# QuentinFuxa/WhisperLiveKit

Measured on AMD Instinct MI355X. Metric: audio seconds transcribed per second (1/RTF), Whisper-base EN simul_whisper AlignAtt, 0.5 s chunks, higher is better.
Workload: dtype f32; 1 GPU; base.en simul_whisper, 1 stream(s) over 1 GPU(s) (1 per GPU), 30 s 16 kHz speech-like stream, 0.5 s chunks, beam 1, frame_threshold 25, seeded random weights, synthetic vocabulary; model=base.en, streams_total=1

## Files before the change

### include/wlk_hip.h

```cpp
#ifndef WLK_HIP_H
#define WLK_HIP_H

#include <stdint.h>

#ifdef __cplusplus
extern "C" {
#endif

#define WLK_OK 0
#define WLK_ERR_ARG (-1)
#define WLK_ERR_HIP (-2)
#define WLK_ERR_STATE (-3)
#define WLK_ERR_CAPACITY (-4)

typedef struct wlk_model wlk_model;
typedef struct wlk_session wlk_session;

typedef struct wlk_dims {
    int32_t n_mels, n_audio_ctx, n_audio_state, n_audio_head, n_audio_layer;
    int32_t n_vocab, n_text_ctx, n_text_state, n_text_head, n_text_layer;
} wlk_dims;

const char* wlk_last_error(void);
int wlk_abi_version(void);
// ... 420 lines not shown
    float scale;
    int64_t lda, ldr, ldc, kv_layer_off, cache_stride;
    int64_t a_floats, w_floats, bias_floats, ln_floats, r_floats, c_floats, cache_floats;
    int64_t a_off[8], c_off[8], r_off[8];
    float* a;
    float* w;
    float* bias;
    float* ln_gamma;
    float* ln_beta;
    float* r;
    float* c;
    float* kcache;
    float* vcache;
} wlk_diag_linear_args;
int wlk_diag_linear_ex(const wlk_diag_linear_args* args);
int wlk_diag_gemv_variant(int m, int n, int k, int has_ln, int kv_mode, char* out_text, int cap);
#define WLK_ENC_X3_GEMM 0
#define WLK_ENC_LN 1
#define WLK_ENC_ATTENTION 2
#define WLK_ENC_PACK 3
typedef struct wlk_diag_enc_op_args {
    int32_t kind, form, m, n, k, n_head, flags, scale_cols, scale_period, r_is_c, x3_out, batch, vt_col0;
    float scale;
    int64_t ld_in, ld_out, ld_out3, ldr, vt_off, vt_ld, bias_off;
    int64_t in_floats, in3_elems, w_floats, bias_floats, r_floats, out_floats, out3_elems;
    int64_t in_off[8], in3_off[8], r_off[8], out_off[8], out3_off[8];
    float* in;
    uint16_t* in3;
    float* w;
    float* bias;
// ... 53 lines not shown
```

### whisperlivekit_amd/_lib.py

```python
from __future__ import annotations

import ctypes as C
import os
import threading
from typing import Optional


_LIB_NAME = "libwlk_hip.so"
_lock = threading.Lock()
_lib: Optional[C.CDLL] = None


class WlkError(RuntimeError):
    """Raised for every non-zero status of the C ABI (message from wlk_last_error())."""


class Dims(C.Structure):
    _fields_ = [(n, C.c_int32) for n in (
        "n_mels", "n_audio_ctx", "n_audio_state", "n_audio_head", "n_audio_layer",
        "n_vocab", "n_text_ctx", "n_text_state", "n_text_head", "n_text_layer")]


class SfDims(C.Structure):
    _fields_ = [(n, C.c_int32) for n in (
# ... 300 lines not shown
        "wlk_diag_env_refresh": (cint, []),
        "wlk_diag_linear_x3": (cint, [p, p, p, cint, cint, cint, cint, C.c_float, cint, p]),
        "wlk_diag_linear_x3_time": (cint, [cint, cint, cint, cint, cint, C.POINTER(C.c_float)]),
        "wlk_diag_layernorm_x3": (cint, [p, p, p, cint, cint, p]),
        "wlk_diag_encoder_attention_x3": (cint, [p, cint, cint, cint, p]),
        "wlk_diag_encoder_attention_x3_time": (cint, [cint, cint, cint, cint, C.POINTER(C.c_float)]),
        "wlk_diag_qkv_x3_attention": (cint, [p, p, p, cint, cint, cint, C.c_float, p, p]),
        "wlk_diag_select": (cint, [C.POINTER(DiagSelectArgs)]),
        "wlk_diag_dec_attention": (cint, [C.POINTER(DiagDecAttentionArgs)]),
        "wlk_diag_topk": (cint, [p, i32, i32, i32, i32, p, p]),
        "wlk_diag_nllb_align": (cint, [p, i32, i32, i32, i32, i32, i32, p, p, p, p]),
        "wlk_diag_nllb_align_rows": (cint, [p, i32, i32, i32, p, p, p, p, p, p, p, p]),
        "wlk_diag_sf_kernel": (cint, [C.POINTER(DiagSfKernelArgs)]),
        "wlk_diag_linear_ex": (cint, [C.POINTER(DiagLinearArgs)]),
        "wlk_diag_gemv_variant": (cint, [cint, cint, cint, cint, cint, C.c_char_p, cint]),
        "wlk_diag_enc_op": (cint, [C.POINTER(DiagEncOpArgs)]),
        "wlk_diag_x3_plan": (cint, [cint, cint, cint, cint, cint, C.c_char_p, cint]),
        "wlk_diag_word_align": (cint, [C.POINTER(DiagWordAlignArgs)]),
        "wlk_diag_nllb_cross_ragged": (cint, [C.POINTER(DiagNllbCrossRaggedArgs)]),
        "wlk_model_set_cif": (cint, [p, p, cint, C.c_float]),
        "wlk_cif_result": (cint, [p, C.POINTER(CifOut)]),
        "wlk_diag_cif": (cint, [p, cint, cint, p, C.c_float, cint, cint, p, p, p]),
    }
    for name, (res, args) in sig.items():
        try:
            fn = getattr(lib, name)
        except AttributeError:
            if "WLK_HIP_LIB" in os.environ and name.startswith("wlk_diag_"):
                continue
            raise
# ... 26 lines not shown
    "wlk_dtw", "wlk_encode_mel", "wlk_log_mel", "wlk_find_alignment",
    "wlk_nllb_arena_floats", "wlk_nllb_tensor_lookup", "wlk_nllb_tensor_name", "wlk_nllb_create", "wlk_nllb_upload",
    "wlk_nllb_finalize", "wlk_nllb_destroy", "wlk_nllb_session_create", "wlk_nllb_session_destroy", "wlk_nllb_encode",
    "wlk_nllb_decode", "wlk_nllb_step", "wlk_nllb_kv_reorder", "wlk_nllb_topk", "wlk_nllb_export", "wlk_nllb_sync",
    "wlk_nllb_step_beam", "wlk_nllb_session_beam_stats",
    "wlk_nllb_session_set_align", "wlk_nllb_step_align", "wlk_nllb_generate_alignatt", "wlk_nllb_session_align_stats",
    "wlk_nllb_batch_create", "wlk_nllb_batch_destroy", "wlk_nllb_batch_encode", "wlk_nllb_batch_step", "wlk_nllb_batch_release",
    "wlk_nllb_batch_export", "wlk_nllb_batch_cross_attention", "wlk_nllb_batch_sync",
    "wlk_nllb_batch_set_align", "wlk_nllb_batch_prefill", "wlk_nllb_batch_step_align", "wlk_nllb_batch_align_stats",
    "wlk_diag_last_error", "wlk_diag_linear", "wlk_diag_linear_time", "wlk_diag_linear_ln", "wlk_diag_layernorm",
    "wlk_diag_encoder_attention", "wlk_diag_encoder_attention_time", "wlk_diag_wave_ops", "wlk_diag_env_refresh",
    "wlk_diag_linear_x3", "wlk_diag_linear_x3_time", "wlk_diag_layernorm_x3",
    "wlk_diag_encoder_attention_x3", "wlk_diag_encoder_attention_x3_time", "wlk_diag_qkv_x3_attention",
    "wlk_diag_select", "wlk_diag_dec_attention", "wlk_diag_topk", "wlk_diag_sf_kernel", "wlk_diag_nllb_align",
    "wlk_diag_nllb_align_rows", "wlk_diag_linear_ex", "wlk_diag_gemv_variant", "wlk_diag_enc_op",
    "wlk_diag_x3_plan", "wlk_diag_word_align", "wlk_diag_nllb_cross_ragged",
    "wlk_model_set_cif", "wlk_cif_result", "wlk_diag_cif",
    "wlk_group_create", "wlk_group_destroy", "wlk_group_step_pick", "wlk_group_stats", "wlk_group_export_logits",
    "wlk_diag_pick_rows",
)


def load() -> C.CDLL:
    global _lib
    if _lib is not None:
        return _lib
    with _lock:
        if _lib is None:
            path = lib_path()
            if not os.path.exists(path):
# ... 27 lines not shown
```

### whisperlivekit_amd/csrc/api.hip

```cpp
#include <cmath>
#include <cstdio>
#include <cstdlib>
#include <atomic>
#include <chrono>
#include <cstring>
#include <map>
#include <memory>
#include <mutex>
#include <string>
#include <vector>

#include "../../include/wlk_hip.h"
#include "common.h"
#include "internal.h"

namespace wlk {

namespace {
struct UtilStream {
    std::mutex mu;
    hipStream_t stream = nullptr;
};
UtilStream g_util[64];
UtilStream& util_of_current_device() {
// ... 413 lines not shown
        s->datt = dev_alloc<float>(R * d);
        s->dq = dev_alloc<float>(R * d);
        s->dmlp = dev_alloc<float>(R * 4 * d);
        const size_t cache = (size_t)D.n_text_layer * beam * ctx * d;
        s->kcache[0] = dev_alloc<float>(cache);
        s->vcache[0] = dev_alloc<float>(cache);
        s->hsel = dev_alloc<float>((size_t)2 * beam * d);
        s->logits_last = dev_alloc<float>((size_t)2 * beam * V);
        s->logits_sot = s->logits_last + (size_t)beam * V;
        s->ring_row = s->step_in + R;
        s->beam_of_row = s->step_in + 2 * R;
        s->d_offset = s->step_in + 3 * R;
        s->ring_rows = (int)ctx + kAlignWindow;
        if (m->n_align > 0) s->ring = dev_alloc<float>((size_t)m->n_align * beam * s->ring_rows * T);
        s->xsplit = dev_alloc<float>(cross_split_scratch_floats(8, D.n_text_head, (int)T));
        s->fsplit = dev_alloc<float>(flash_split_scratch_floats(s->max_rows, D.n_text_head, wlk_session::kFlashSplitsMax));
        s->z = dev_alloc<float>((size_t)beam * std::max(m->n_align, 1) * T + (size_t)beam * 128);
        s->attn_last = dev_alloc_zero<float>((size_t)beam * T, st);
        s->adj_row = dev_alloc<int>(3 * wlk_session::kAdjCap);
        s->src_rows = dev_alloc<int>(8);
        if (beam >= 2 && beam <= 7) s->anc = dev_alloc_zero<unsigned char>((size_t)beam * ctx, st);
        s->top_vals = dev_alloc<float>((size_t)beam * 18);
        s->top_ids = reinterpret_cast<int*>(s->top_vals) + (size_t)beam * 8;
        s->frames = s->top_ids + (size_t)beam * 8;
        WLK_HIP(hipMalloc(&s->topk_scratch, topk_scratch_bytes(beam)));
        s->probs = dev_alloc<float>(beam);
        WLK_HIP(hipHostMalloc(&s->pinned, wlk_session::kPinnedBytes, hipHostMallocDefault));
        WLK_HIP(hipHostMalloc(&s->dec_stage, 65536, hipHostMallocDefault));
        WLK_HIP(hipHostMalloc(&s->audio_stage, wlk_session::kPinnedBytes, hipHostMallocDefault));
        WLK_HIP(hipEventCreateWithFlags(&s->audio_stage_ev, hipEventDisableTiming));
// ... 16 lines not shown
        return WLK_OK;
    });
}

int wlk_session_destroy(wlk_session* s) {
    if (!s) return WLK_OK;
    if (s->step_count && getenv("WLK_STEP_TIMING"))
        fprintf(stderr, "[wlk] one-replay steps: %llu, mean %.1f us per step (graph launch call %.1f us)\n",
                (unsigned long long)s->step_count, s->step_ns / 1e3 / s->step_count, s->step_launch_ns / 1e3 / s->step_count);
    (void)wlk_engine_detach(s);
    (void)hipSetDevice(s->m->device);
    (void)hipStreamSynchronize(s->stream);
    float* fl[] = {s->audio[0], s->audio[1], s->logmel, s->frame_max, s->logmel_alt, s->frame_max_alt, s->mel_t, s->x1p, s->ex, s->eh, s->eqkv,
                   s->eatt, s->emlp, s->enc_out, s->cross_kv, s->dx, s->dh, s->dqkv, s->datt, s->dq, s->dmlp,
                   s->kcache[0], s->kcache[1], s->vcache[0], s->vcache[1], s->hsel, s->logits_last,
                   s->ring, s->z, s->attn_last, s->qk_debug, s->xsplit, s->fsplit, s->top_vals, s->probs};
    for (float* p : fl)
        if (p) (void)hipFree(p);
    int* il[] = {s->step_in, s->adj_row, s->src_rows};
    for (int* p : il)
        if (p) (void)hipFree(p);
    for (auto& e : s->step_exec)
        if (e) (void)hipGraphExecDestroy(e);
    for (auto& e : s->bstep_exec)
        if (e) (void)hipGraphExecDestroy(e);
    if (s->anc) (void)hipFree(s->anc);
    if (s->topk_scratch) (void)hipFree(s->topk_scratch);
    if (s->pcm16_dev) (void)hipFree(s->pcm16_dev);
    if (s->eh3) (void)hipFree(s->eh3);
    if (s->eqkv3) (void)hipFree(s->eqkv3);
    if (s->enc_out3) (void)hipFree(s->enc_out3);
// ... 465 lines not shown
        if (fused) {
            g.A = s->dx; g.ln_gamma = L.ln1w; g.ln_beta = L.ln1b;
            g.kcache = kc; g.vcache = vc; g.kv_pos = s->d_offset; g.kv_d = d; g.kv_ctx = ctx_len;
            launch_gemv(c, g, "dec_ln1_qkv_kv");
        } else {
            launch_layernorm(c, s->dx, d, L.ln1w, L.ln1b, s->dh, d, R, d, "dec_ln1");
            g.A = s->dh;
            if (!gemv_applicable(R, d) && gemm_takes_kwave(R, 3 * d, d)) {
                g.kcache = kc; g.vcache = vc; g.kv_pos = s->d_offset; g.kv_d = d; g.kv_ctx = ctx_len; g.kv_ntok = n_tok;
                launch_gemm(c, g, "dec_qkv");
            } else {
                launch_linear(c, g, "dec_qkv");
                launch_kv_append(c, s->dqkv, kc, vc, n_rows, n_tok, s->d_offset, d, ctx_len);
            }
        }
        if (ancestry)
            launch_decoder_self_attention_anc(c, s->dqkv, kc, vc, s->anc, s->datt, n_rows, s->d_offset, d, H, ctx_len);
        else
            launch_decoder_self_attention(c, s->dqkv, kc, vc, s->datt, n_rows, n_tok, s->d_offset, d, H, ctx_len);
        GemmArgs o;
        o.A = s->datt; o.lda = d; o.W = L.outw; o.bias = L.outb; o.C = s->dx; o.ldc = d; o.M = R; o.N = d; o.K = d;
        o.flags = kGemmResidual; o.R = s->dx; o.ldr = d;
        launch_linear(c, o, "dec_out");

        GemmArgs q;
        q.lda = d; q.W = L.xqw; q.bias = L.xqb; q.C = s->dq; q.ldc = d; q.M = R; q.N = d; q.K = d;
        q.flags = kGemmScaleCols; q.scale = scale; q.scale_cols = d;
        const bool fold_xq = fused && R == 1 && !s->debug && !s->align_raw_scores && cross_split_folds_query(d);
        if (fold_xq) {
        } else if (fused) {
            q.A = s->dx; q.ln_gamma = L.lnxw; q.ln_beta = L.lnxb;
            launch_gemv(c, q, "dec_lnx_xq");
        } else {
            launch_layernorm(c, s->dx, d, L.lnxw, L.lnxb, s->dh, d, R, d, "dec_lnx");
            q.A = s->dh;
            launch_linear(c, q, "dec_xq");
        }
        const int* ranks_l = m->n_align > 0 ? m->head_rank + (size_t)i * H : nullptr;
        bool merged_xout = false;
        GemmArgs xo_mg;
        if ((R > 8 || s->align_raw_scores) && !s->debug) {
            if (fold_xq) throw std::logic_error("decode: the folded query projection left no q for the flash kernel");
            FlashArgs fa;
// ... 15 lines not shown
            ca.q = s->dq;
            ca.k = s->cross_kv + (size_t)i * 2 * d;
            ca.v = ca.k + d;
            ca.ldkv = (long)D.n_text_layer * 2 * d;
            ca.out = s->datt;
            ca.rows = R; ca.d = d; ca.n_head = H; ca.T = T;
            ca.head_rank = ranks_l;
            ca.ring = s->ring;
            ca.ring_row = s->ring_row;
            ca.beam_of_row = s->beam_of_row;
            ca.ring_rows = s->ring_rows;
            ca.n_beam = s->beam;
            ca.qk_debug = s->debug ? s->qk_debug + (size_t)i * s->max_rows * H * T : nullptr;
            if (fold_xq) {
                ca.xq_x = s->dx; ca.xq_w = L.xqw; ca.xq_b = L.xqb; ca.xq_gamma = L.lnxw; ca.xq_beta = L.lnxb; ca.xq_scale = scale;
            }
            if (R <= 8 && !s->debug) {
                float* sc = s->xsplit;
                float* pm = sc + (size_t)8 * H * T;
                float* pl = pm + (size_t)8 * H * 8;
                float* po = pl + (size_t)8 * H * 8;
                merged_xout = fused && R == 1 && gemv1_folds_merge(d);
                launch_decoder_cross_attention_split(c, ca, sc, pm, pl, po, !merged_xout);
                if (merged_xout) {
                    xo_mg.mg_pm = pm; xo_mg.mg_pl = pl; xo_mg.mg_po = po; xo_mg.mg_scores = sc;
                    xo_mg.mg_head_rank = ranks_l; xo_mg.mg_ring = s->ring; xo_mg.mg_ring_row = s->ring_row;
                    xo_mg.mg_side_heads = m->layer_heads + (size_t)i * H;
                    xo_mg.mg_beam_of_row = s->beam_of_row; xo_mg.mg_heads = H; xo_mg.mg_T = T;
                    xo_mg.mg_ring_rows = s->ring_rows; xo_mg.mg_n_beam = s->beam;
                    xo_mg.mg_side_blocks = ranks_l ? m->layer_rank_count[i] : 0;
                }
            } else {
                launch_decoder_cross_attention(c, ca);
            }
        }
        GemmArgs xo = xo_mg;
        xo.A = s->datt; xo.lda = d; xo.W = L.xoutw; xo.bias = L.xoutb; xo.C = s->dx; xo.ldc = d; xo.M = R; xo.N = d;
        xo.K = d; xo.flags = kGemmResidual; xo.R = s->dx; xo.ldr = d;
        launch_linear(c, xo, "dec_xout");
        transformer_mlp(c, L, s->dx, s->dh, s->dmlp, R, d, "dec_ln2", "dec_fc1", "dec_fc2");
    }
    if (scores_dumped && m->n_align > 0 && !s->align_raw_scores)
        launch_ring_softmax(c, s->ring, s->ring_row, s->beam_of_row, m->all_ranks, m->n_align, R, s->ring_rows, s->beam, T);
    GemmArgs lg;
    lg.lda = d; lg.W = m->w_tok_emb; lg.C = s->logits_last; lg.ldc = V; lg.M = n_rows; lg.N = V; lg.K = d;
    if (side_align && !fused) throw std::logic_error("decode: side workgroups need the fused step");
    if (fused) {
        lg.A = s->dx; lg.ln_gamma = m->w_ln_w; lg.ln_beta = m->w_ln_b;
        lg.side_align = side_align; lg.side_blocks = side_blocks; lg.side_zf = side_zf;
        launch_gemv(c, lg, "dec_lnf_logits");
    } else if (first && n_rows == 1 && gemv_applicable(2, d) && getenv("WLK_NO_PREFILL_MERGE") == nullptr) {
        launch_layernorm(c, s->dx + (size_t)(n_tok - 1) * d, (long)(sot_index - (n_tok - 1)) * d, m->w_ln_w, m->w_ln_b,
                         s->hsel, d, 2, d, "dec_ln_f");
// ... 831 lines not shown
```

### whisperlivekit_amd/csrc/common.h

```cpp
#pragma once
#include <hip/hip_runtime.h>

#include <cstdint>
#include <stdexcept>
#include <mutex>
#include <string>

namespace wlk {

constexpr int kNFft = 400;
constexpr int kHop = 160;
constexpr int kNFreq = 201;
constexpr int kMelFrames = 3000;
constexpr int kPadSamples = 480000;
constexpr int kHeadDim = 64;
constexpr int kAlignWindow = 16;

struct HipError : std::runtime_error {
    using std::runtime_error::runtime_error;
};

inline void hip_check(hipError_t e, const char* what, const char* file, int line) {
    if (e != hipSuccess) {
        throw HipError(std::string(what) + " failed: " + hipGetErrorString(e) + " (" + file + ":" +
// ... 360 lines not shown
void launch_embed_rows(const LaunchCtx& ctx, const StepRow* rows, const float* tok_emb, const float* pos_emb, float* x,
                       int n_rows, int d);
void launch_decoder_self_attention_rows(const LaunchCtx& ctx, const float* qkv, const StepRow* rows, long layer_off,
                                        float* out, int n_rows, int d, int n_head, int ctx_len);
void launch_kv_append(const LaunchCtx& ctx, const float* qkv, float* kc, float* vc, int n_rows, int n_tok,
                      const int* offset_dev, int d, int ctx_len);
void launch_kv_append_rows(const LaunchCtx& ctx, const float* qkv, const StepRow* rows, long layer_off, int n_rows, int d);
void launch_decoder_self_attention_anc(const LaunchCtx& ctx, const float* qkv, const float* kc, const float* vc,
                                       const unsigned char* anc, float* out, int n_rows, const int* offset, int d,
                                       int n_head, int ctx_len);
void launch_anc_update(const LaunchCtx& ctx, unsigned char* anc, const int* ctl, const int* offset, int n_rows, int ctx_len);
void launch_anc_update_block(const LaunchCtx& ctx, unsigned char* anc, const int* block, int n_rows, int ctx_len);
void launch_decoder_self_attention(const LaunchCtx& ctx, const float* qkv, const float* kc, const float* vc,
                                   float* out, int n_rows, int n_tok, const int* offset_dev, int d, int n_head,
                                   int ctx_len);
struct CrossAttnArgs {
    const float* q;
    const float* k;
    const float* v;
    long ldkv;
    float* out;
    int rows, d, n_head, T;
    const int* head_rank;
    float* ring;
    const int* ring_row;
    const int* beam_of_row;
    int ring_rows, n_beam;
    float* qk_debug;
    const StepRow* step_rows = nullptr;
    long kv_off = 0;
    const float* xq_x = nullptr;
    const float* xq_w = nullptr;
    const float* xq_b = nullptr;
    const float* xq_gamma = nullptr;
    const float* xq_beta = nullptr;
    float xq_scale = 1.f;
};
void launch_decoder_cross_attention(const LaunchCtx& ctx, const CrossAttnArgs& a);
bool cross_split_folds_query(int d);
void launch_decoder_cross_attention_split(const LaunchCtx& ctx, const CrossAttnArgs& a, float* scores, float* pm,
                                          float* pl, float* po, bool merge = true);
constexpr int kCrossSplitWays = 8;
size_t cross_split_scratch_floats(int rows, int n_head, int T);
void launch_kv_gather(const LaunchCtx& ctx, const float* src, float* dst, const int* source_rows, int n_rows,
                      int len, int d, int ctx_len, int n_layer);

inline int sf_sub_len(int n) { return (n - 1) / 2 + 1; }
void launch_sf_scale_copy(const LaunchCtx& ctx, const float* src, float* dst, long n, float scale);
constexpr int kSfMaxSegments = 8;
struct SfSegments {
    int n = 0;
// ... 113 lines not shown
```

### whisperlivekit_amd/csrc/decoder.hip

```cpp
#include <cstddef>

#include <cstdlib>

#include "common.h"
#include "wave_ops.h"

namespace wlk {

__global__ __launch_bounds__(128) void embed_kernel(const int* __restrict__ tokens,
                                                    const float* __restrict__ tok_emb,
                                                    const float* __restrict__ pos_emb, float* __restrict__ x,
                                                    int n_tok, const int* __restrict__ offset_p, int d) {
    const int row = blockIdx.x;
    const int p = row % n_tok;
    const int offset = *offset_p;
    const float* e = tok_emb + (long)tokens[row] * d;
    const float* pe = pos_emb + (long)(offset + p) * d;
    for (int c = threadIdx.x; c < d; c += 128) x[(long)row * d + c] = e[c] + pe[c];
}

void launch_embed(const LaunchCtx& ctx, const int* tokens, const float* tok_emb, const float* pos_emb,
                  float* x, int n_rows, int n_tok, const int* offset, int d) {
    KernelScope ks(ctx, "dec_embed");
    hipLaunchKernelGGL(embed_kernel, dim3(n_rows * n_tok), dim3(128), 0, ctx.stream, tokens, tok_emb, pos_emb, x,
// ... 280 lines not shown
                       layer_off, (const unsigned char*)nullptr);
    WLK_HIP(hipGetLastError());
}

void launch_decoder_self_attention_anc(const LaunchCtx& ctx, const float* qkv, const float* kc, const float* vc,
                                       const unsigned char* anc, float* out, int n_rows, const int* offset, int d,
                                       int n_head, int ctx_len) {
    if (ctx_len > 448 + 64) throw std::invalid_argument("self-attention: context too long");
    if (n_rows < 1 || n_rows > 8 || !anc) throw std::invalid_argument("ancestry self-attention: 1..8 rows and a table");
    KernelScope ks(ctx, "dec_self_attention");
    hipLaunchKernelGGL(decoder_self_attention_kernel<true>, dim3(n_rows, n_head), dim3(256), 0, ctx.stream, qkv, kc, vc,
                       (const StepRow*)nullptr, offset, d, ctx_len, 1, out, 0L, anc);
    WLK_HIP(hipGetLastError());
}

__global__ __launch_bounds__(512) void anc_update_kernel(unsigned char* __restrict__ anc, const int* __restrict__ ctl,
                                                         const int* __restrict__ offset_p, int n_rows, int ctx_len) {
    const int t = threadIdx.x;
    if (t >= ctx_len) return;
    const int offset = *offset_p;
    const bool fresh = ctl[7] != 0;
    int col[7];
#pragma unroll
    for (int b = 0; b < 7; ++b) col[b] = b < n_rows ? (fresh ? b : (int)anc[(long)b * ctx_len + t]) : 0;
#pragma unroll
    for (int b = 0; b < 7; ++b) {
        if (b >= n_rows) break;
        const int sb = ctl[b];
        int v = b;
        if (t < offset) {
// ... 158 lines not shown
    WLK_HIP(hipGetLastError());
}

constexpr int kCrossSplit = 8;
static_assert(kCrossSplit == kCrossSplitWays, "gemv1's merged operand load assumes the same split count");
constexpr int kCrossUnroll = 12;

struct CrossSplitRest {
    long kv_off;
    const float* xq_x;
    const float* xq_w;
    const float* xq_b;
    const float* xq_gamma;
    const float* xq_beta;
    float xq_scale;
};
template <int UB>
__global__ __launch_bounds__(256) void cross_split_kernel(const float* __restrict__ k_in, const float* __restrict__ v_in,
                                                          const float* __restrict__ q_in, long ldkv, int T, int d, int n_head,
                                                          const StepRow* __restrict__ step_rows,
                                                          float* __restrict__ scores, float* __restrict__ pm,
                                                          float* __restrict__ pl, float* __restrict__ po, CrossSplitRest a) {
    __shared__ __attribute__((aligned(16))) float qs[64];
    __shared__ float sc[kCrossUnroll * 16];
    __shared__ float red[8];
    __shared__ __attribute__((aligned(16))) float part[16 * 64];
    const int tid = threadIdx.x, lane = tid & 63, wave = tid >> 6;
    const int row = blockIdx.x, head = blockIdx.y, ks = blockIdx.z;
    const int sub = lane & 15, kq = lane >> 4;
    const int chunk = (T + kCrossSplit - 1) / kCrossSplit;
    const int k_lo = ks * chunk, k_hi = min(T, k_lo + chunk);
    const gcf_ptr kbase = to_global(step_rows ? step_rows[row].cross_kv + a.kv_off : k_in);
// ... 8 lines not shown
    const gcf_ptr k_first = kb + (long)j0 * ldkv, k_safe = kb + (long)k_lo * ldkv;
    const long v_minus_k = vb - kb;
    float4 kk[kCrossUnroll];
#pragma unroll
    for (int u = 0; u < kCrossUnroll; ++u) {
        kk[u] = ldg4(j0 + 16 * u < k_hi ? k_first + u * row_step : k_safe);
    }
    float4 vv[kCrossUnroll];
#pragma unroll
    for (int u = 0; u < kCrossUnroll; ++u)
        vv[u] = ldg4((j0 + 16 * u < k_hi ? k_first + u * row_step : k_safe) + v_minus_k);
    if constexpr (UB != 0) {
        const int K = d, K4 = K >> 2;
        const float* xrow = a.xq_x + (long)row * K;
        constexpr int NPASS = 32 / UB;
        float4 x[UB], ga[UB], be[UB];
        float v[UB * 4];
        float4 w[NPASS][UB];
#pragma unroll
        for (int u = 0; u < UB; ++u) {
            const int c = lane + 64 * u;
            const int cc = (c < K4 ? c : 0) * 4;
            x[u] = *reinterpret_cast<const float4*>(xrow + cc);
            ga[u] = *reinterpret_cast<const float4*>(a.xq_gamma + cc);
            be[u] = *reinterpret_cast<const float4*>(a.xq_beta + cc);
        }
#pragma unroll
        for (int i = 0; i < UB * 4; ++i) {
            const int c = lane + 64 * i;
            v[i] = xrow[c < K ? c : 0];
        }
        const float bias_l = (a.xq_b ? a.xq_b + head * 64 + wave * 16 + (lane & 15) : xrow)[0];
        auto load_rows = [&](int i0) {
#pragma unroll
            for (int r = 0; r < NPASS; ++r) {
                const int n = head * 64 + wave * 16 + i0 + r;
#pragma unroll
                for (int u = 0; u < UB; ++u) {
                    const int c = lane + 64 * u;
                    w[r][u] = *reinterpret_cast<const float4*>(a.xq_w + (long)n * K + (c < K4 ? c : 0) * 4);
                }
            }
        };
        load_rows(0);
        {
            float sum = 0.f;
#pragma unroll
            for (int i = 0; i < UB * 4; ++i) {
                v[i] = (lane + 64 * i) < K ? v[i] : 0.f;
                sum += v[i];
            }
            sum = wave_sum(sum);
            const float mean = sum / (float)K;
            float sq = 0.f;
#pragma unroll
            for (int i = 0; i < UB * 4; ++i) {
                const float t = (lane + 64 * i) < K ? v[i] - mean : 0.f;
                sq += t * t;
            }
            sq = wave_sum(sq);
            const float rstd = 1.0f / sqrtf(sq / (float)K + 1e-5f);
#pragma unroll
            for (int u = 0; u < UB; ++u) {
                x[u].x = (x[u].x - mean) * rstd * ga[u].x + be[u].x;
                x[u].y = (x[u].y - mean) * rstd * ga[u].y + be[u].y;
                x[u].z = (x[u].z - mean) * rstd * ga[u].z + be[u].z;
                x[u].w = (x[u].w - mean) * rstd * ga[u].w + be[u].w;
            }
        }
#pragma unroll
        for (int i0 = 0; i0 < 16; i0 += NPASS) {
            if (i0 > 0) load_rows(i0);
#pragma unroll
            for (int r = 0; r < NPASS; ++r) {
                float acc = 0.f;
#pragma unroll
// ... 98 lines not shown
                         ? a.step_rows[row].ring + ((long)rank * a.ring_rows + a.step_rows[row].ring_row) * a.T
                         : a.ring + (((long)rank * a.n_beam + a.beam_of_row[row]) * a.ring_rows + a.ring_row[row]) * a.T;
        const float* srow = scores + ((long)row * a.n_head + head) * a.T;
        for (int j = tid; j < a.T; j += 256) dst[j] = expf(srow[j] - M) / L;
    }
}

void launch_decoder_cross_attention_split(const LaunchCtx& ctx, const CrossAttnArgs& a, float* scores, float* pm,
                                          float* pl, float* po, bool merge) {
    if ((a.T + kCrossSplit - 1) / kCrossSplit > kCrossUnroll * 16) throw std::invalid_argument("cross-attention: T too large");
    if ((kCrossSplit - 1) * ((a.T + kCrossSplit - 1) / kCrossSplit) >= a.T)
        throw std::invalid_argument("cross-attention: T too small for the key split (a slice would hold no key)");
    {
        KernelScope ks(ctx, "dec_cross_split", 4.0 * a.rows * (double)a.T * a.d, 4.0 * 2.0 * a.rows * (double)a.T * a.d);
        const dim3 grid(a.rows, a.n_head, kCrossSplit);
        const CrossSplitRest rest{a.kv_off, a.xq_x, a.xq_w, a.xq_b, a.xq_gamma, a.xq_beta, a.xq_scale};
#define WLK_CROSS_SPLIT(UBv)                                                                                              \
    hipLaunchKernelGGL(cross_split_kernel<UBv>, grid, dim3(256), 0, ctx.stream, a.k, a.v, a.q, a.ldkv, a.T, a.d, a.n_head, \
                       a.step_rows, scores, pm, pl, po, rest)
        if (a.xq_w) {
            if (a.d % 256 != 0 || a.d < 256 || a.d > 2048) throw std::invalid_argument("cross-attention: cannot fold the query projection");
            const int ub = a.d / 256;
            if (ub <= 2) WLK_CROSS_SPLIT(2);
            else if (ub <= 4) WLK_CROSS_SPLIT(4);
            else WLK_CROSS_SPLIT(8);
        } else {
            WLK_CROSS_SPLIT(0);
        }
#undef WLK_CROSS_SPLIT
        WLK_HIP(hipGetLastError());
    }
    if (merge) {
        KernelScope ks(ctx, "dec_cross_merge");
        hipLaunchKernelGGL(cross_merge_kernel, dim3(a.rows, a.n_head), dim3(256), 0, ctx.stream, a, scores, pm, pl, po);
        WLK_HIP(hipGetLastError());
    }
}
bool cross_split_folds_query(int d) {
// ... 33 lines not shown
```

### whisperlivekit_amd/csrc/diag.hip

```cpp
#include <cstdio>
#include <cmath>
#include <cstdlib>
#include <cstring>
#include <stdexcept>
#include <string>
#include <vector>

#include "../../include/wlk_hip.h"
#include "common.h"
#include "internal.h"
#include "nllb_internal.h"
#include "wave_ops.h"

using namespace wlk;

namespace {
thread_local std::string g_diag_error;
struct DevBuf {
    float* p = nullptr;
    explicit DevBuf(size_t n, const float* host = nullptr) {
        WLK_HIP(hipMalloc(reinterpret_cast<void**>(&p), std::max<size_t>(n, 1) * sizeof(float)));
        if (host) WLK_HIP(hipMemcpy(p, host, n * sizeof(float), hipMemcpyHostToDevice));
    }
    ~DevBuf() { (void)hipFree(p); }
// ... 68 lines not shown
                    int64_t ldr, int m, int n, int k, int flags, float scale, int scale_cols, int force_gemv, float* c) {
    return run([&]() {
        DevBuf A(a_floats, a), W((size_t)n * k, w), B(n, bias), R(r ? (size_t)m * ldr : 1, r), Cc((size_t)m * n);
        GemmArgs g;
        g.A = A.p; g.lda = lda; g.W = W.p; g.bias = bias ? B.p : nullptr; g.C = Cc.p; g.ldc = n;
        g.R = r ? R.p : nullptr; g.ldr = ldr; g.M = m; g.N = n; g.K = k; g.flags = flags; g.scale = scale;
        g.scale_cols = scale_cols;
        LaunchCtx ctx;
        g.force_kwave = force_gemv == 2;
        g.force_kernel = (force_gemv >= 2 && force_gemv <= 4) || (force_gemv >= 6 && force_gemv <= 8) ? force_gemv : 0;
        if (force_gemv == 1) launch_gemv(ctx, g, "diag_gemv");
        else if (force_gemv >= 5 && force_gemv <= 8) launch_gemm_kp(ctx, g, "diag_gemm_kp");
        else launch_gemm(ctx, g, "diag_gemm");
        WLK_HIP(hipDeviceSynchronize());
        WLK_HIP(hipMemcpy(c, Cc.p, (size_t)m * n * sizeof(float), hipMemcpyDeviceToHost));
    });
}

int wlk_diag_linear_time(int m, int n, int k, int flags, int force, int reps, float* us_per_launch) {
    return run([&]() {
        std::vector<float> ha((size_t)m * k), hw((size_t)n * k);
        unsigned seed = 12345u;
        auto rnd = [&]() { seed = seed * 1664525u + 1013904223u; return ((seed >> 8) & 0xffff) / 65536.0f - 0.5f; };
        for (auto& v : ha) v = rnd();
        for (auto& v : hw) v = rnd() * 0.05f;
        DevBuf A((size_t)m * k, ha.data()), W((size_t)n * k, hw.data()), B(n), R((size_t)m * n), Cc((size_t)m * n);
        WLK_HIP(hipMemset(B.p, 0, n * sizeof(float)));
        WLK_HIP(hipMemset(R.p, 0, (size_t)m * n * sizeof(float)));
        GemmArgs g;
        g.A = A.p; g.lda = k; g.W = W.p; g.bias = B.p; g.C = Cc.p; g.ldc = n; g.R = (flags & kGemmResidual) ? R.p : nullptr;
// ... 1536 lines not shown
```

### whisperlivekit_amd/csrc/internal.h

```cpp
#pragma once
#include <algorithm>
#include <map>
#include <memory>
#include <chrono>
#include <cstdlib>
#include <thread>
#include <mutex>
#include <stdexcept>
#include <string>
#include <vector>

#include "../../include/wlk_hip.h"
#include "common.h"

namespace wlk {

const std::string& get_last_error();

template <typename F>
inline int guarded(F&& f) {
    try {
        return f();
    } catch (const HipError& e) {
        set_last_error(e.what());
// ... 164 lines not shown
    float* vcache[2] = {nullptr, nullptr};
    int kv_cur = 0;
    int self_len = 0;
    int n_steps = 0;
    int prefill_rows = 0;
    int last_rows = 0, last_ntok = 0;
    float *hsel = nullptr, *logits_last = nullptr, *logits_sot = nullptr;
    bool have_sot = false;
    int* step_in = nullptr;
    int *ring_row = nullptr, *beam_of_row = nullptr, *d_offset = nullptr;
    float* ring = nullptr;
    int ring_rows = 0;
    float *z = nullptr, *attn_last = nullptr;
    float* qk_debug = nullptr;
    float* xsplit = nullptr;
    float* fsplit = nullptr;
    static constexpr int kFlashSplitsMax = 16;
    static int flash_splits();

    int *adj_row = nullptr, *src_rows = nullptr;
    float* top_vals = nullptr;
    void* topk_scratch = nullptr;
    int *top_ids = nullptr, *frames = nullptr;
    float* probs = nullptr;
    static constexpr int kAdjCap = 4096;
    void* pinned = nullptr;
    static constexpr size_t kPinnedBytes = 1 << 20;
    void* dec_stage = nullptr;
    hipEvent_t dec_stage_ev = nullptr;
    bool dec_stage_used = false;
// ... 115 lines not shown
```

Before: 208.4 audio_s/s.

## Fuse decoder self-attention with output projection and fold the merge into cross-split

For single-row greedy decoding, a new kernel computes each head's self-attention and immediately multiplies it by that head's slice of the output projection, writing per-head partial outputs. The cross-attention split kernel then sums the head partials with the bias and residual, writes the post-self-attention row, and applies the layer norm for the folded query projection. This drops the separate dec_out GEMM launch and the round trip through the attention buffer. In exchange, every cross-split block re-reads the head partials, and the new attention kernel recomputes softmax per output column tile (grid z = d/32).

Result: no change. 208.8 audio_s/s, median of 3 (+0.2%).

```diff
diff --git a/include/wlk_hip.h b/include/wlk_hip.h
--- a/include/wlk_hip.h
+++ b/include/wlk_hip.h
@@ -458,6 +458,8 @@
     float* vcache;
 } wlk_diag_linear_args;
 int wlk_diag_linear_ex(const wlk_diag_linear_args* args);
+int wlk_diag_self_attention_proj(const float* qkv, const float* kcache, const float* vcache, const float* wo, const float* bias,
+                                 const float* resid, int offset, int d, int n_head, int ctx_len, float* partials, float* merged);
 int wlk_diag_gemv_variant(int m, int n, int k, int has_ln, int kv_mode, char* out_text, int cap);
 #define WLK_ENC_X3_GEMM 0
 #define WLK_ENC_LN 1
diff --git a/whisperlivekit_amd/_lib.py b/whisperlivekit_amd/_lib.py
--- a/whisperlivekit_amd/_lib.py
+++ b/whisperlivekit_amd/_lib.py
@@ -338,6 +338,7 @@
         "wlk_diag_sf_kernel": (cint, [C.POINTER(DiagSfKernelArgs)]),
         "wlk_diag_linear_ex": (cint, [C.POINTER(DiagLinearArgs)]),
         "wlk_diag_gemv_variant": (cint, [cint, cint, cint, cint, cint, C.c_char_p, cint]),
+        "wlk_diag_self_attention_proj": (cint, [p, p, p, p, p, p, cint, cint, cint, cint, p, p]),
         "wlk_diag_enc_op": (cint, [C.POINTER(DiagEncOpArgs)]),
         "wlk_diag_x3_plan": (cint, [cint, cint, cint, cint, cint, C.c_char_p, cint]),
         "wlk_diag_word_align": (cint, [C.POINTER(DiagWordAlignArgs)]),
@@ -394,6 +395,7 @@
     "wlk_diag_encoder_attention_x3", "wlk_diag_encoder_attention_x3_time", "wlk_diag_qkv_x3_attention",
     "wlk_diag_select", "wlk_diag_dec_attention", "wlk_diag_topk", "wlk_diag_sf_kernel", "wlk_diag_nllb_align",
     "wlk_diag_nllb_align_rows", "wlk_diag_linear_ex", "wlk_diag_gemv_variant", "wlk_diag_enc_op",
+    "wlk_diag_self_attention_proj",
     "wlk_diag_x3_plan", "wlk_diag_word_align", "wlk_diag_nllb_cross_ragged",
     "wlk_model_set_cif", "wlk_cif_result", "wlk_diag_cif",
     "wlk_group_create", "wlk_group_destroy", "wlk_group_step_pick", "wlk_group_stats", "wlk_group_export_logits",
diff --git a/whisperlivekit_amd/csrc/api.hip b/whisperlivekit_amd/csrc/api.hip
--- a/whisperlivekit_amd/csrc/api.hip
+++ b/whisperlivekit_amd/csrc/api.hip
@@ -451,6 +451,7 @@
         s->ring_rows = (int)ctx + kAlignWindow;
         if (m->n_align > 0) s->ring = dev_alloc<float>((size_t)m->n_align * beam * s->ring_rows * T);
         s->xsplit = dev_alloc<float>(cross_split_scratch_floats(8, D.n_text_head, (int)T));
+        if (beam == 1) s->sfold = dev_alloc<float>(((size_t)D.n_text_head + 1) * d);
         s->fsplit = dev_alloc<float>(flash_split_scratch_floats(s->max_rows, D.n_text_head, wlk_session::kFlashSplitsMax));
         s->z = dev_alloc<float>((size_t)beam * std::max(m->n_align, 1) * T + (size_t)beam * 128);
         s->attn_last = dev_alloc_zero<float>((size_t)beam * T, st);
@@ -497,7 +498,7 @@
     float* fl[] = {s->audio[0], s->audio[1], s->logmel, s->frame_max, s->logmel_alt, s->frame_max_alt, s->mel_t, s->x1p, s->ex, s->eh, s->eqkv,
                    s->eatt, s->emlp, s->enc_out, s->cross_kv, s->dx, s->dh, s->dqkv, s->datt, s->dq, s->dmlp,
                    s->kcache[0], s->kcache[1], s->vcache[0], s->vcache[1], s->hsel, s->logits_last,
-                   s->ring, s->z, s->attn_last, s->qk_debug, s->xsplit, s->fsplit, s->top_vals, s->probs};
+                   s->ring, s->z, s->attn_last, s->qk_debug, s->xsplit, s->sfold, s->fsplit, s->top_vals, s->probs};
     for (float* p : fl)
         if (p) (void)hipFree(p);
     int* il[] = {s->step_in, s->adj_row, s->src_rows};
@@ -993,19 +994,25 @@
                 launch_kv_append(c, s->dqkv, kc, vc, n_rows, n_tok, s->d_offset, d, ctx_len);
             }
         }
-        if (ancestry)
-            launch_decoder_self_attention_anc(c, s->dqkv, kc, vc, s->anc, s->datt, n_rows, s->d_offset, d, H, ctx_len);
-        else
-            launch_decoder_self_attention(c, s->dqkv, kc, vc, s->datt, n_rows, n_tok, s->d_offset, d, H, ctx_len);
-        GemmArgs o;
-        o.A = s->datt; o.lda = d; o.W = L.outw; o.bias = L.outb; o.C = s->dx; o.ldc = d; o.M = R; o.N = d; o.K = d;
-        o.flags = kGemmResidual; o.R = s->dx; o.ldr = d;
-        launch_linear(c, o, "dec_out");
+        const bool fold_xq = fused && R == 1 && !s->debug && !s->align_raw_scores && cross_split_folds_query(d);
+        const bool self_fold = fold_xq && !ancestry && !c.prof && s->sfold && L.outb && decoder_self_fold(d, H);
+        float* const x1 = self_fold ? s->sfold + (size_t)H * d : s->dx;
+        if (self_fold) {
+            launch_decoder_self_attention_proj(c, s->dqkv, kc, vc, L.outw, s->sfold, 1, s->d_offset, d, H, ctx_len);
+        } else {
+            if (ancestry)
+                launch_decoder_self_attention_anc(c, s->dqkv, kc, vc, s->anc, s->datt, n_rows, s->d_offset, d, H, ctx_len);
+            else
+                launch_decoder_self_attention(c, s->dqkv, kc, vc, s->datt, n_rows, n_tok, s->d_offset, d, H, ctx_len);
+            GemmArgs o;
+            o.A = s->datt; o.lda = d; o.W = L.outw; o.bias = L.outb; o.C = s->dx; o.ldc = d; o.M = R; o.N = d; o.K = d;
+            o.flags = kGemmResidual; o.R = s->dx; o.ldr = d;
+            launch_linear(c, o, "dec_out");
+        }
 
         GemmArgs q;
         q.lda = d; q.W = L.xqw; q.bias = L.xqb; q.C = s->dq; q.ldc = d; q.M = R; q.N = d; q.K = d;
         q.flags = kGemmScaleCols; q.scale = scale; q.scale_cols = d;
-        const bool fold_xq = fused && R == 1 && !s->debug && !s->align_raw_scores && cross_split_folds_query(d);
         if (fold_xq) {
         } else if (fused) {
             q.A = s->dx; q.ln_gamma = L.lnxw; q.ln_beta = L.lnxb;
@@ -1051,6 +1058,7 @@
             ca.qk_debug = s->debug ? s->qk_debug + (size_t)i * s->max_rows * H * T : nullptr;
             if (fold_xq) {
                 ca.xq_x = s->dx; ca.xq_w = L.xqw; ca.xq_b = L.xqb; ca.xq_gamma = L.lnxw; ca.xq_beta = L.lnxb; ca.xq_scale = scale;
+                if (self_fold) { ca.sf_p = s->sfold; ca.sf_bias = L.outb; ca.sf_x1 = x1; }
             }
             if (R <= 8 && !s->debug) {
                 float* sc = s->xsplit;
@@ -1073,7 +1081,7 @@
         }
         GemmArgs xo = xo_mg;
         xo.A = s->datt; xo.lda = d; xo.W = L.xoutw; xo.bias = L.xoutb; xo.C = s->dx; xo.ldc = d; xo.M = R; xo.N = d;
-        xo.K = d; xo.flags = kGemmResidual; xo.R = s->dx; xo.ldr = d;
+        xo.K = d; xo.flags = kGemmResidual; xo.R = x1; xo.ldr = d;
         launch_linear(c, xo, "dec_xout");
         transformer_mlp(c, L, s->dx, s->dh, s->dmlp, R, d, "dec_ln2", "dec_fc1", "dec_fc2");
     }
diff --git a/whisperlivekit_amd/csrc/common.h b/whisperlivekit_amd/csrc/common.h
--- a/whisperlivekit_amd/csrc/common.h
+++ b/whisperlivekit_amd/csrc/common.h
@@ -398,6 +398,10 @@
 void launch_decoder_self_attention(const LaunchCtx& ctx, const float* qkv, const float* kc, const float* vc,
                                    float* out, int n_rows, int n_tok, const int* offset_dev, int d, int n_head,
                                    int ctx_len);
+bool decoder_self_fold(int d, int n_head);
+void launch_decoder_self_attention_proj(const LaunchCtx& ctx, const float* qkv, const float* kc, const float* vc,
+                                        const float* wo, float* partials, int n_rows, const int* offset_dev, int d,
+                                        int n_head, int ctx_len);
 struct CrossAttnArgs {
     const float* q;
     const float* k;
@@ -419,6 +423,9 @@
     const float* xq_gamma = nullptr;
     const float* xq_beta = nullptr;
     float xq_scale = 1.f;
+    const float* sf_p = nullptr;
+    const float* sf_bias = nullptr;
+    float* sf_x1 = nullptr;
 };
 void launch_decoder_cross_attention(const LaunchCtx& ctx, const CrossAttnArgs& a);
 bool cross_split_folds_query(int d);
diff --git a/whisperlivekit_amd/csrc/decoder.hip b/whisperlivekit_amd/csrc/decoder.hip
--- a/whisperlivekit_amd/csrc/decoder.hip
+++ b/whisperlivekit_amd/csrc/decoder.hip
@@ -318,6 +318,149 @@
     WLK_HIP(hipGetLastError());
 }
 
+__global__ __launch_bounds__(256) void decoder_self_attention_proj_kernel(const float* __restrict__ qkv,
+                                                                          const float* __restrict__ kc_in,
+                                                                          const float* __restrict__ vc_in,
+                                                                          const int* __restrict__ offset_p, int d, int ctx_len,
+                                                                          const float* __restrict__ wo, float* __restrict__ P) {
+    __shared__ float sc[448 + 64];
+    __shared__ float red[8];
+    __shared__ __attribute__((aligned(16))) float part[16 * 64];
+    __shared__ __attribute__((aligned(16))) float oh[64];
+    const int tid = threadIdx.x, lane = tid & 63, wave = tid >> 6;
+    const int sub = lane & 15, kq = lane >> 4;
+    const int row = blockIdx.x;
+    const int head = blockIdx.y;
+    const int n_head = gridDim.y;
+    const float4 q4 = *reinterpret_cast<const float4*>(qkv + (long)row * 3 * d + head * 64 + sub * 4);
+    const int offset = *offset_p;
+    const gcf_ptr kc = to_global(kc_in), vc = to_global(vc_in);
+    const gcf_ptr kb = kc + (long)row * ctx_len * d + head * 64 + sub * 4;
+    const gcf_ptr vb = vc + (long)row * ctx_len * d + head * 64 + sub * 4;
+    float4 kk0[8], vv0[8], wo4[2];
+#pragma unroll
+    for (int u = 0; u < 8; ++u) {
+        const int j = wave * 4 + 16 * u + kq;
+        kk0[u] = ldg4(kb + (long)(j < ctx_len ? j : 0) * d);
+    }
+    const int n0 = (int)blockIdx.z * 32 + wave * 8 + kq;
+#pragma unroll
+    for (int u = 0; u < 2; ++u) wo4[u] = ldg4(to_global(wo) + (long)(n0 + 4 * u) * d + head * 64 + sub * 4);
+    __builtin_amdgcn_sched_barrier(0);
+    const int n_keys = offset + 1;
+#pragma unroll
+    for (int u = 0; u < 8; ++u) {
+        const int j = wave * 4 + 16 * u + kq;
+        vv0[u] = ldg4(vb + (long)(j < n_keys ? j : 0) * d);
+    }
+
+    float mx = -INFINITY;
+    for (int base = wave * 4; base < n_keys; base += 16 * 8) {
+        float4 kk[8];
+#pragma unroll
+        for (int u = 0; u < 8; ++u) {
+            const int j = base + 16 * u + kq;
+            const bool ok = j < n_keys;
+            if (base == wave * 4) kk[u] = kk0[u];
+            else kk[u] = ldg4(kb + (long)(ok ? j : 0) * d);
+        }
+#pragma unroll
+        for (int u = 0; u < 8; ++u) {
+            const int j = base + 16 * u + kq;
+            float acc = 0.f;
+            acc = fmaf(q4.x, kk[u].x, acc);
+            acc = fmaf(q4.y, kk[u].y, acc);
+            acc = fmaf(q4.z, kk[u].z, acc);
+            acc = fmaf(q4.w, kk[u].w, acc);
+            acc = row16_sum_1248(acc);
+            if (j < n_keys) {
+                if (sub == 0) sc[j] = acc;
+                mx = fmaxf(mx, acc);
+            }
+        }
+    }
+    mx = wave_max(mx);
+    if (lane == 0) red[wave] = mx;
+    __syncthreads();
+    mx = fmaxf(fmaxf(red[0], red[1]), fmaxf(red[2], red[3]));
+    float sum = 0.f;
+    for (int j = tid; j < n_keys; j += 256) {
+        const float e = expf(sc[j] - mx);
+        sc[j] = e;
+        sum += e;
+    }
+    sum = wave_sum(sum);
+    if (lane == 0) red[4 + wave] = sum;
+    __syncthreads();
+    sum = (red[4] + red[5]) + (red[6] + red[7]);
+    for (int j = tid; j < n_keys; j += 256) sc[j] = sc[j] / sum;
+    __syncthreads();
+
+    float4 o = make_float4(0.f, 0.f, 0.f, 0.f);
+    for (int base = wave * 4; base < n_keys; base += 16 * 8) {
+        float4 vv[8];
+        float ww[8];
+#pragma unroll
+        for (int u = 0; u < 8; ++u) {
+            const int j = base + 16 * u + kq;
+            const bool ok = j < n_keys;
+            if (base == wave * 4) vv[u] = vv0[u];
+            else vv[u] = ldg4(vb + (long)(ok ? j : 0) * d);
+            ww[u] = ok ? sc[j] : 0.f;
+        }
+#pragma unroll
+        for (int u = 0; u < 8; ++u) {
+            o.x = fmaf(ww[u], vv[u].x, o.x);
+            o.y = fmaf(ww[u], vv[u].y, o.y);
+            o.z = fmaf(ww[u], vv[u].z, o.z);
+            o.w = fmaf(ww[u], vv[u].w, o.w);
+        }
+    }
+    asm volatile("" ::"v"(q4.x), "v"(q4.y), "v"(q4.z), "v"(q4.w));
+#pragma unroll
+    for (int u = 0; u < 8; ++u) {
+        asm volatile("" ::"v"(kk0[u].x), "v"(kk0[u].y), "v"(kk0[u].z), "v"(kk0[u].w));
+        asm volatile("" ::"v"(vv0[u].x), "v"(vv0[u].y), "v"(vv0[u].z), "v"(vv0[u].w));
+    }
+    reinterpret_cast<float4*>(part)[(wave * 4 + kq) * 16 + sub] = o;
+    __syncthreads();
+    if (tid < 64) {
+        float acc = 0.f;
+#pragma unroll
+        for (int s = 0; s < 16; ++s) acc += part[s * 64 + tid];
+        oh[tid] = acc;
+    }
+    __syncthreads();
+    const float4 o4 = reinterpret_cast<const float4*>(oh)[sub];
+    float* prow = P + ((long)row * n_head + head) * d;
+#pragma unroll
+    for (int u = 0; u < 2; ++u) {
+        float acc = 0.f;
+        acc = fmaf(wo4[u].x, o4.x, acc);
+        acc = fmaf(wo4[u].y, o4.y, acc);
+        acc = fmaf(wo4[u].z, o4.z, acc);
+        acc = fmaf(wo4[u].w, o4.w, acc);
+        acc = row16_sum_1248(acc);
+        if (sub == 0) prow[n0 + 4 * u] = acc;
+    }
+}
+
+bool decoder_self_fold(int d, int n_head) {
+    if (getenv("WLK_NO_SELF_FOLD") != nullptr) return false;
+    return d % 256 == 0 && d >= 256 && d <= 512 && n_head * 64 == d && cross_split_folds_query(d);
+}
+
+void launch_decoder_self_attention_proj(const LaunchCtx& ctx, const float* qkv, const float* kc, const float* vc,
+                                        const float* wo, float* partials, int n_rows, const int* offset, int d, int n_head,
+                                        int ctx_len) {
+    if (ctx_len > 448 + 64) throw std::invalid_argument("self-attention: context too long");
+    if (d % 32 != 0 || n_head * 64 != d || n_rows < 1) throw std::invalid_argument("fused self-attention: d = 64 n_head");
+    KernelScope ks(ctx, "dec_self_attention_proj");
+    hipLaunchKernelGGL(decoder_self_attention_proj_kernel, dim3(n_rows, n_head, d / 32), dim3(256), 0, ctx.stream, qkv, kc,
+                       vc, offset, d, ctx_len, wo, partials);
+    WLK_HIP(hipGetLastError());
+}
+
 __global__ __launch_bounds__(512) void anc_update_kernel(unsigned char* __restrict__ anc, const int* __restrict__ ctl,
                                                          const int* __restrict__ offset_p, int n_rows, int ctx_len) {
     const int t = threadIdx.x;
@@ -506,8 +649,24 @@
     const float* xq_gamma;
     const float* xq_beta;
     float xq_scale;
+    const float* sf_p;
+    const float* sf_bias;
+    float* sf_x1;
 };
-template <int UB>
+
+template <int H>
+__device__ __forceinline__ float4 merge_head_partials(const float4 (&p)[H], float4 bias, float4 resid) {
+    float4 s = p[0];
+#pragma unroll
+    for (int h = 1; h < H; ++h) {
+        s.x += p[h].x; s.y += p[h].y; s.z += p[h].z; s.w += p[h].w;
+    }
+    s.x += bias.x; s.y += bias.y; s.z += bias.z; s.w += bias.w;
+    s.x += resid.x; s.y += resid.y; s.z += resid.z; s.w += resid.w;
+    return s;
+}
+
+template <int UB, int SFH = 0>
 __global__ __launch_bounds__(256) void cross_split_kernel(const float* __restrict__ k_in, const float* __restrict__ v_in,
                                                           const float* __restrict__ q_in, long ldkv, int T, int d, int n_head,
                                                           const StepRow* __restrict__ step_rows,
@@ -546,8 +705,11 @@
         const int K = d, K4 = K >> 2;
         const float* xrow = a.xq_x + (long)row * K;
         constexpr int NPASS = 32 / UB;
+        constexpr bool SF = SFH > 0;
+        constexpr int HM = SF ? SFH : 1;
         float4 x[UB], ga[UB], be[UB];
-        float v[UB * 4];
+        [[maybe_unused]] float v[UB * 4];
+        [[maybe_unused]] float4 sp[UB][HM], sb[UB];
         float4 w[NPASS][UB];
 #pragma unroll
         for (int u = 0; u < UB; ++u) {
@@ -556,11 +718,19 @@
             x[u] = *reinterpret_cast<const float4*>(xrow + cc);
             ga[u] = *reinterpret_cast<const float4*>(a.xq_gamma + cc);
             be[u] = *reinterpret_cast<const float4*>(a.xq_beta + cc);
-        }
-#pragma unroll
-        for (int i = 0; i < UB * 4; ++i) {
-            const int c = lane + 64 * i;
-            v[i] = xrow[c < K ? c : 0];
+            if constexpr (SF) {
+                sb[u] = *reinterpret_cast<const float4*>(a.sf_bias + cc);
+#pragma unroll
+                for (int h = 0; h < HM; ++h)
+                    sp[u][h] = *reinterpret_cast<const float4*>(a.sf_p + ((long)row * HM + h) * K + cc);
+            }
+        }
+        if constexpr (!SF) {
+#pragma unroll
+            for (int i = 0; i < UB * 4; ++i) {
+                const int c = lane + 64 * i;
+                v[i] = xrow[c < K ? c : 0];
+            }
         }
         const float bias_l = (a.xq_b ? a.xq_b + head * 64 + wave * 16 + (lane & 15) : xrow)[0];
         auto load_rows = [&](int i0) {
@@ -575,23 +745,58 @@
             }
         };
         load_rows(0);
+        if constexpr (SF) {
+#pragma unroll
+            for (int u = 0; u < UB; ++u) pin_loaded(sp[u][0]);
+            __builtin_amdgcn_sched_barrier(0);
+        }
         {
-            float sum = 0.f;
-#pragma unroll
-            for (int i = 0; i < UB * 4; ++i) {
-                v[i] = (lane + 64 * i) < K ? v[i] : 0.f;
-                sum += v[i];
+            float mean, rstd;
+            if constexpr (SF) {
+#pragma unroll
+                for (int u = 0; u < UB; ++u) x[u] = merge_head_partials<HM>(sp[u], sb[u], x[u]);
+                if (head == 0 && ks == 0 && wave == 0) {
+#pragma unroll
+                    for (int u = 0; u < UB; ++u)
+                        if (lane + 64 * u < K4) *reinterpret_cast<float4*>(a.sf_x1 + (long)row * K + (lane + 64 * u) * 4) = x[u];
+                }
+                float sum = 0.f;
+#pragma unroll
+                for (int u = 0; u < UB; ++u) {
+                    if (lane + 64 * u < K4) {
+                        sum += x[u].x; sum += x[u].y; sum += x[u].z; sum += x[u].w;
+                    }
+                }
+                sum = wave_sum(sum);
+                mean = sum / (float)K;
+                float sq = 0.f;
+#pragma unroll
+                for (int u = 0; u < UB; ++u) {
+                    if (lane + 64 * u < K4) {
+                        const float tx = x[u].x - mean, ty = x[u].y - mean, tz = x[u].z - mean, tw = x[u].w - mean;
+                        sq += tx * tx; sq += ty * ty; sq += tz * tz; sq += tw * tw;
+                    }
+                }
+                sq = wave_sum(sq);
+                rstd = 1.0f / sqrtf(sq / (float)K + 1e-5f);
+            } else {
+                float sum = 0.f;
+#pragma unroll
+                for (int i = 0; i < UB * 4; ++i) {
+                    v[i] = (lane + 64 * i) < K ? v[i] : 0.f;
+                    sum += v[i];
+                }
+                sum = wave_sum(sum);
+                mean = sum / (float)K;
+                float sq = 0.f;
+#pragma unroll
+                for (int i = 0; i < UB * 4; ++i) {
+                    const float t = (lane + 64 * i) < K ? v[i] - mean : 0.f;
+                    sq += t * t;
+                }
+                sq = wave_sum(sq);
+                rstd = 1.0f / sqrtf(sq / (float)K + 1e-5f);
             }
-            sum = wave_sum(sum);
-            const float mean = sum / (float)K;
-            float sq = 0.f;
-#pragma unroll
-            for (int i = 0; i < UB * 4; ++i) {
-                const float t = (lane + 64 * i) < K ? v[i] - mean : 0.f;
-                sq += t * t;
-            }
-            sq = wave_sum(sq);
-            const float rstd = 1.0f / sqrtf(sq / (float)K + 1e-5f);
 #pragma unroll
             for (int u = 0; u < UB; ++u) {
                 x[u].x = (x[u].x - mean) * rstd * ga[u].x + be[u].x;
@@ -720,14 +925,18 @@
     {
         KernelScope ks(ctx, "dec_cross_split", 4.0 * a.rows * (double)a.T * a.d, 4.0 * 2.0 * a.rows * (double)a.T * a.d);
         const dim3 grid(a.rows, a.n_head, kCrossSplit);
-        const CrossSplitRest rest{a.kv_off, a.xq_x, a.xq_w, a.xq_b, a.xq_gamma, a.xq_beta, a.xq_scale};
-#define WLK_CROSS_SPLIT(UBv)                                                                                              \
-    hipLaunchKernelGGL(cross_split_kernel<UBv>, grid, dim3(256), 0, ctx.stream, a.k, a.v, a.q, a.ldkv, a.T, a.d, a.n_head, \
-                       a.step_rows, scores, pm, pl, po, rest)
+        const CrossSplitRest rest{a.kv_off, a.xq_x, a.xq_w, a.xq_b, a.xq_gamma, a.xq_beta, a.xq_scale, a.sf_p, a.sf_bias, a.sf_x1};
+#define WLK_CROSS_SPLIT(...)                                                                                                   \
+    hipLaunchKernelGGL((cross_split_kernel<__VA_ARGS__>), grid, dim3(256), 0, ctx.stream, a.k, a.v, a.q, a.ldkv, a.T, a.d,      \
+                       a.n_head, a.step_rows, scores, pm, pl, po, rest)
+        if (a.sf_p && (!a.xq_w || !a.sf_bias || !a.sf_x1 || (a.d != 256 && a.d != 512) || a.n_head * 64 != a.d || a.sf_x1 == a.xq_x))
+            throw std::invalid_argument("cross-attention: the split-form row needs the folded query projection, d = 64 n_head = 256 or 512, a bias and a row of its own to write");
         if (a.xq_w) {
             if (a.d % 256 != 0 || a.d < 256 || a.d > 2048) throw std::invalid_argument("cross-attention: cannot fold the query projection");
             const int ub = a.d / 256;
-            if (ub <= 2) WLK_CROSS_SPLIT(2);
+            if (a.sf_p && a.n_head == 8) WLK_CROSS_SPLIT(2, 8);
+            else if (a.sf_p) WLK_CROSS_SPLIT(2, 4);
+            else if (ub <= 2) WLK_CROSS_SPLIT(2);
             else if (ub <= 4) WLK_CROSS_SPLIT(4);
             else WLK_CROSS_SPLIT(8);
         } else {
diff --git a/whisperlivekit_amd/csrc/diag.hip b/whisperlivekit_amd/csrc/diag.hip
--- a/whisperlivekit_amd/csrc/diag.hip
+++ b/whisperlivekit_amd/csrc/diag.hip
@@ -106,6 +106,45 @@
         else launch_gemm(ctx, g, "diag_gemm");
         WLK_HIP(hipDeviceSynchronize());
         WLK_HIP(hipMemcpy(c, Cc.p, (size_t)m * n * sizeof(float), hipMemcpyDeviceToHost));
+    });
+}
+
+int wlk_diag_self_attention_proj(const float* qkv, const float* kcache, const float* vcache, const float* wo, const float* bias,
+                                 const float* resid, int offset, int d, int n_head, int ctx_len, float* partials, float* merged) {
+    try {
+        if (!qkv || !kcache || !vcache || !wo || !bias || !resid || !partials || !merged)
+            throw std::invalid_argument("wlk_diag_self_attention_proj: null arguments");
+        if (d % 256 != 0 || d < 256 || d > 512 || n_head * 64 != d)
+            throw std::invalid_argument("wlk_diag_self_attention_proj: d = 64 n_head, a multiple of 256 up to 512");
+        if (ctx_len < 1 || ctx_len > 512 || offset < 0 || offset >= ctx_len)
+            throw std::invalid_argument("wlk_diag_self_attention_proj: offset < ctx_len <= 512");
+    } catch (const std::invalid_argument& e) {
+        g_diag_error = e.what();
+        return WLK_ERR_ARG;
+    }
+    return run([&]() {
+        constexpr int T = 64;
+        const size_t cache = (size_t)ctx_len * d, D = d;
+        DevBuf QKV(3 * D, qkv), KC(cache, kcache), VC(cache, vcache), WO(D * D, wo), B(D, bias), X(D, resid), P(n_head * D), X1(D);
+        DevBuf KV(T * 2 * D), WQ(D * D), LN(2 * D), SCR(cross_split_scratch_floats(1, n_head, T)), OFF(1);
+        WLK_HIP(hipMemcpy(OFF.p, &offset, sizeof(int), hipMemcpyHostToDevice));
+        WLK_HIP(hipMemset(KV.p, 0, T * 2 * D * sizeof(float)));
+        WLK_HIP(hipMemset(WQ.p, 0, D * D * sizeof(float)));
+        WLK_HIP(hipMemset(LN.p, 0, 2 * D * sizeof(float)));
+        LaunchCtx ctx;
+        launch_decoder_self_attention_proj(ctx, QKV.p, KC.p, VC.p, WO.p, P.p, 1, reinterpret_cast<const int*>(OFF.p), d, n_head, ctx_len);
+        CrossAttnArgs ca{};
+        ca.k = KV.p; ca.v = KV.p + D; ca.ldkv = 2 * d; ca.rows = 1; ca.d = d; ca.n_head = n_head; ca.T = T;
+        ca.xq_x = X.p; ca.xq_w = WQ.p; ca.xq_gamma = LN.p; ca.xq_beta = LN.p + D; ca.xq_scale = 1.f;
+        ca.sf_p = P.p; ca.sf_bias = B.p; ca.sf_x1 = X1.p;
+        float* sc = SCR.p;
+        float* pm = sc + (size_t)n_head * T;
+        float* pl = pm + (size_t)n_head * kCrossSplitWays;
+        float* po = pl + (size_t)n_head * kCrossSplitWays;
+        launch_decoder_cross_attention_split(ctx, ca, sc, pm, pl, po, false);
+        WLK_HIP(hipDeviceSynchronize());
+        WLK_HIP(hipMemcpy(partials, P.p, n_head * D * sizeof(float), hipMemcpyDeviceToHost));
+        WLK_HIP(hipMemcpy(merged, X1.p, D * sizeof(float), hipMemcpyDeviceToHost));
     });
 }
 
diff --git a/whisperlivekit_amd/csrc/internal.h b/whisperlivekit_amd/csrc/internal.h
--- a/whisperlivekit_amd/csrc/internal.h
+++ b/whisperlivekit_amd/csrc/internal.h
@@ -202,6 +202,7 @@
     float *z = nullptr, *attn_last = nullptr;
     float* qk_debug = nullptr;
     float* xsplit = nullptr;
+    float* sfold = nullptr;
     float* fsplit = nullptr;
     static constexpr int kFlashSplitsMax = 16;
     static int flash_splits();
```
